# TonyLianLong/RCF-UnsupVideoSeg

Hardware: AMD Instinct MI355X
Metric: training frames/sec at 480x854 (RCF stage-1) (higher is better)
Workload: dtype f32 (3xfp16-MFMA split); 1 GPU; RCF stage-1 ResNet50+FCN train step, 8 pairs/GPU 480x854 RGB+flow, fp32, SyncBN, Adam (configs[1]); pairs_per_gpu=8, global_pairs=8, parallelism=dp1

## Files before the change

### include/rcf_hip.h

```cpp
#ifndef RCF_HIP_H
#define RCF_HIP_H
#include <stddef.h>
#include <stdint.h>

#ifdef __cplusplus
extern "C" {
#endif

#define RCF_EINVAL (-1)
#define RCF_EWORKSPACE (-2)

#define RCF_F32 0
#define RCF_BF16 1

const char *rcf_version(void);

typedef struct {
    int N, H, W, Cin;
    int Ho, Wo, Cout;
    int R, S, stride, pad, dil;
    int x_pitch, y_pitch;
    const unsigned *amax_x, *amax_w, *amax_dy;
    const void *w_pairs;
    const void *w_pairs_t;
// ... 212 lines not shown
                         const unsigned char *relu_mask, const double *sums2, const double *sums2_local, double count,
                         float *dgamma, float *dbeta, unsigned *amax_out, const unsigned *amax_x, const unsigned *amax_dy,
                         const rcf_bn_bwd_second *second, unsigned flags, void *stream);
int rcf_bn_bwd_reduce_mp(const void *dy, int ydt, int dy_pitch, const void *x, int xdt, int x_pitch, const void *y,
                         int y_pitch, long rows, int C, const float *mean, const float *invstd, int relu,
                         const unsigned char *relu_mask, const float *chan_scale, long rows_per_image, double *sums2,
                         void *workspace, size_t workspace_bytes, unsigned flags, void *stream);
int rcf_bn_bwd_apply_mp(const void *dy, int ydt, int dy_pitch, const void *x, int xdt, int x_pitch, const void *y,
                        int y_pitch, void *dx, int dx_pitch, void *dres, int dres_pitch, int res_beta, long rows, int C,
                        const float *mean, const float *invstd, const float *gamma, int relu,
                        const unsigned char *relu_mask, const float *chan_scale, long rows_per_image,
                        const double *sums2, const double *sums2_local, double count, float *dgamma, float *dbeta,
                        unsigned *amax_out, const unsigned *amax_x, const unsigned *amax_dy, unsigned flags, void *stream);
int rcf_colsum_mp(const void *x, int xdt, long rows, int C, int pitch, float *out, int beta, void *workspace,
                  size_t workspace_bytes, void *stream);

int rcf_maxpool3x3s2_fwd_f32(const float *x, float *y, uint8_t *argmax, int N, int H, int W, int C, int Ho,
                             int Wo, void *stream);
int rcf_maxpool3x3s2_bwd_f32(const float *dy, const uint8_t *argmax, float *dx, int N, int H, int W, int C,
                             int Ho, int Wo, void *stream);
int rcf_resize_bilinear_nhwc_fwd_f32(const float *x, int x_pitch, float *y, int y_pitch, int N, int Hi, int Wi,
                                     int Ho, int Wo, int C, int align_corners, void *stream);
int rcf_resize_bilinear_nhwc_bwd_f32(const float *dy, int dy_pitch, float *dx, int dx_pitch, int beta, int N,
                                     int Hi, int Wi, int Ho, int Wo, int C, int align_corners, void *stream);
int rcf_resize_bilinear_nhwc_fwd_frame_f32(const float *x, int x_pitch, float *y, int y_pitch, int N, int Hi, int Wi,
                                           int Ho, int Wo, int C, int align_corners, int frame, void *stream);
int rcf_resize_bilinear_nhwc_bwd_frame_f32(const float *dy, int dy_pitch, float *dx, int dx_pitch, int beta, int N,
                                           int Hi, int Wi, int Ho, int Wo, int C, int align_corners, int frame,
                                           void *stream);
int rcf_resize_bilinear_nchw_f32(const float *x, float *y, int planes, int Hi, int Wi, int Ho, int Wo,
// ... 184 lines not shown
```

### rcf-unsupvideoseg_amd/_lib.py

```python
import ctypes
import os
from ctypes import c_int, c_uint, c_long, c_float, c_double, c_void_p, c_size_t, c_char_p

HERE = os.path.dirname(os.path.abspath(__file__))
LIB_PATH = os.path.join(HERE, "librcf_hip.so")
LIB_PATHS = {"bf16": LIB_PATH, "f16": os.path.join(HERE, "librcf_hip_f16.so")}
ACTIVE = "bf16"


class RcfHipError(RuntimeError):
    pass


class ConvShape(ctypes.Structure):
    _fields_ = [(n, c_int) for n in ("N", "H", "W", "Cin", "Ho", "Wo", "Cout", "R", "S", "stride", "pad", "dil",
                                     "x_pitch", "y_pitch")] + \
               [(n, ctypes.c_void_p) for n in ("amax_x", "amax_w", "amax_dy", "w_pairs", "w_pairs_t", "w_pairs2",
                                                "w_pairs2_t", "amax_y")] + \
               [("flags", ctypes.c_uint), ("struct_bytes", ctypes.c_uint)]


class BnBwdIn(ctypes.Structure):
    _fields_ = [("x", ctypes.c_void_p), ("x_pitch", c_int), ("relu_mask", ctypes.c_void_p), ("mean", ctypes.c_void_p),
                ("invstd", ctypes.c_void_p)]
# ... 170 lines not shown
    "rcf_fill_f32": (c_int, [P, c_long, c_float, P]),
    "rcf_dropout2d_scale_f32": (c_int, [P, c_long, c_float, ctypes.c_ulonglong, P]),
    "rcf_bn_stats_mp": (c_int, [P, c_int, c_long, c_int, c_int, P, P, c_size_t, P]),
    "rcf_bn_apply_mp": (c_int, [P, c_int, c_int, P, c_int, P, c_int, c_int, c_long, c_int, P, P, P, P, c_int, P, c_long, P,
                                P, P, P, P, c_uint, P]),
    "rcf_bn_apply_res_mp": (c_int, [P, c_int, c_int, P, c_int, P, P, c_int, c_int, c_long, c_int, P, P, P, P, c_int, P, c_long, P,
                                    P, P, P, P, c_uint, P]),
    "rcf_bn_bwd_reduce2_mp": (c_int, [P, c_int, c_int, P, c_int, c_int, P, c_int, c_long, c_int, P, P, P, P, P, P, P, c_size_t, c_uint, P]),
    "rcf_bn_bwd_apply2_mp": (c_int, [P, c_int, c_int, P, c_int, c_int, P, c_int, c_long, c_int, P, P, P, P, P, P, c_double, P, P, P, P, P, P,
                                     c_uint, P]),
    "rcf_bn_bwd_reduce_mp": (c_int, [P, c_int, c_int, P, c_int, c_int, P, c_int, c_long, c_int, P, P, c_int, P, P, c_long,
                                     P, P, c_size_t, c_uint, P]),
    "rcf_bn_bwd_apply_mp": (c_int, [P, c_int, c_int, P, c_int, c_int, P, c_int, P, c_int, P, c_int, c_int, c_long, c_int, P,
                                    P, P, c_int, P, P, c_long, P, P, c_double, P, P, P, P, P, c_uint, P]),
    "rcf_colsum_mp": (c_int, [P, c_int, c_long, c_int, c_int, P, c_int, P, c_size_t, P]),
    "rcf_maxpool3x3s2_fwd_mp": (c_int, [P, P, c_int, P, c_int, c_int, c_int, c_int, c_int, c_int, P]),
    "rcf_maxpool3x3s2_bwd_mp": (c_int, [P, P, P, c_int, c_int, c_int, c_int, c_int, c_int, c_int, P]),
    "rcf_resize_bilinear_nhwc_fwd_mp": (c_int, [P, c_int, P, c_int, c_int, c_int, c_int, c_int, c_int, c_int, c_int, c_int,
                                                c_int, P]),
    "rcf_resize_bilinear_nhwc_bwd_mp": (c_int, [P, c_int, P, c_int, c_int, c_int, c_int, c_int, c_int, c_int, c_int, c_int,
                                                c_int, c_int, P]),
    "rcf_copy2d_batched_mp": (c_int, [P, c_long, c_long, c_long, P, c_long, c_long, c_long, c_int, c_long, c_int, c_int,
                                      c_int, c_int, P]),
    "rcf_copy2d_mp": (c_int, [P, c_int, c_long, P, c_int, c_long, c_long, c_int, c_int, P]),
    "rcf_split_rect_mp": (c_int, [P, P, P, c_int, c_int, c_int, c_int, c_int, c_int, c_int, c_int, c_int, P]),
    "rcf_conv_weight_bf16_bytes": (c_size_t, [c_int, c_int, c_int, c_int, c_int]),
    "rcf_conv_weight_bf16": (c_int, [P, c_int, c_int, c_int, c_int, c_int, P, c_uint, P]),
    "rcf_conv2d_fwd_stats_bf16_workspace_bytes": (c_size_t, [_CS]),
    "rcf_conv2d_fwd_bf16": (c_int, [P, P, P, P, c_int, _CS, _CR, c_int, c_float, c_int, P, P, c_size_t, P]),
    "rcf_conv2d_dgrad_bf16_workspace_bytes": (c_size_t, [_CS]),
# ... 63 lines not shown
```

### rcf-unsupvideoseg_amd/backbone.py

```python
import torch
import torch.nn as nn

from . import layers, ops
from .layers import (Act, BatchNorm2d, Conv2d, commuted_concat_conv, commuted_concat_conv_ok, concat_channels,
                     maxpool3x3s2)


def make_norm(norm_cfg, n):
    t = (norm_cfg or {}).get("type", "BN")
    if t not in ("BN", "SyncBN"):
        raise NotImplementedError(f"norm type {t}")
    return BatchNorm2d(n, requires_grad=bool((norm_cfg or {}).get("requires_grad", True)), sync=(t == "SyncBN"))


class Downsample(nn.Module):

    def __init__(self, conv, norm):
        super().__init__()
        self.add_module("0", conv)
        self.add_module("1", norm)

    def fwd(self, x, tape, dist, lazy=False):
        conv, norm = getattr(self, "0"), getattr(self, "1")
        if layers.fold_ok(conv, norm, x):
# ... 90 lines not shown
        if pretrained is not None:
            raise NotImplementedError("load checkpoints through load_state_dict (main.py:76-144 does)")
        for m in self.modules():
            if isinstance(m, Conv2d):
                nn.init.kaiming_normal_(m.weight, a=0, mode="fan_out", nonlinearity="relu")
            elif isinstance(m, BatchNorm2d):
                nn.init.constant_(m.weight, 1)
                nn.init.constant_(m.bias, 0)
        if self.zero_init_residual:
            for m in self.modules():
                if isinstance(m, Bottleneck):
                    nn.init.constant_(m.bn3.weight, 0)

    def fwd(self, img, tape, dist=None):
        tape.mark("stem")
        x = self.bn1.fwd(self.conv1.fwd(img, tape, stats=self.bn1.stats_request(dist)), tape, relu=True, dist=dist)
        x = maxpool3x3s2(x, tape)
        outs = []
        for i in range(self.num_stages):
            tape.mark(f"layer{i + 1}")
            nxt = getattr(getattr(self, f"layer{i + 2}"), "0").takes_planes(tape.act_dtype) if i + 1 < self.num_stages else self.heads_take_planes
            x = getattr(self, f"layer{i + 1}").fwd(x, tape, dist, next_takes_planes=nxt)
            if i in self.out_indices:
                outs.append(x)
        return outs

    def forward(self, x):
        from .layers import Tape
        img = Act(ops.nchw_to_nhwc(x.contiguous().float(), 4), needs_grad=False)
        outs = self.fwd(img, Tape(enabled=False))
        return tuple(ops.nhwc_to_nchw(o.t) for o in outs)

# ... 86 lines not shown
```

### rcf-unsupvideoseg_amd/config.py

```python
import argparse
import os

import yaml


class _UniqueKeyLoader(yaml.SafeLoader):
    def construct_mapping(self, node, deep=False):
        seen = set()
        for key_node, _ in node.value:
            key = self.construct_object(key_node, deep=deep)
            if key in seen:
                raise ValueError(f"Duplicate {key!r} key found in YAML.")
            seen.add(key)
        return super().construct_mapping(node, deep)


def _merge(base, new):
    for k, v in new.items():
        if isinstance(v, dict) and isinstance(base.get(k), dict):
            _merge(base[k], v)
        else:
            base[k] = v
    return base

# ... 122 lines not shown
        if name == "stage22_soft":
            kw["pl_mask_pos_th"] = -1
        oc = 2
    elif name == "freeze":
        kw = stage1_model_kwargs(ms, dropout=0.0, norm=norm)
        kw["freeze_backbone"] = True
    else:
        raise KeyError(name)
    kw.update(log_interval=10 ** 9, train_iter=1)
    return kw, oc


class Schedule:

    __slots__ = ("overlap_wgrad", "late_wgrad", "side_priority", "overlap_teacher", "fuse_bn_stats", "fuse_bn_finalize",
                 "fuse_bn_bwd", "relu_bitmask", "defer_residual", "lazy_downsample_norm", "merge_downsample_bwd", "fold_bn", "fold_max_k", "fold_masked_dgrad", "fp16_pairs",
                 "h2_kinds", "planes", "join_planes", "nt_stores", "bf16_stem", "autocast_fp16_as_bf16", "cache_weight_operands", "bulk_weight_prep", "grad_group",
                 "teacher_group")

    def __init__(self):
        self.overlap_wgrad = self.late_wgrad = self.overlap_teacher = True
        self.side_priority = 0
        self.fuse_bn_stats = self.fuse_bn_finalize = self.relu_bitmask = self.defer_residual = self.lazy_downsample_norm = True
        self.merge_downsample_bwd = True
        self.fuse_bn_bwd = False
        self.fold_bn, self.fold_max_k, self.fold_masked_dgrad = True, 512, True
        self.fp16_pairs, self.h2_kinds, self.planes, self.join_planes = True, "fdw", True, "stage"
        self.bf16_stem = self.cache_weight_operands = self.bulk_weight_prep = True
        self.grad_group, self.teacher_group = "auto", False
        self.nt_stores = 0
        self.autocast_fp16_as_bf16 = False

    def set(self, **kw):
        old = {k: getattr(self, k) for k in kw}
        for k, v in kw.items():
            setattr(self, k, v)
        return old

    def parse(self, items):
# ... 11 lines not shown
```

### rcf-unsupvideoseg_amd/csrc/bn.hip

```cpp
#include "rcf_common.h"

#include <type_traits>

namespace {

constexpr int RED_THREADS = 256;

struct Sweep {
    int mode, group;
    long band;
    __device__ __forceinline__ long positions(long rows) const { return mode ? 8 * band : rows; }
    __device__ __forceinline__ long row(long l) const {
        if (!mode) return l;
        const long g = l / group, w = l - g * group;
        const long b = g & 7, pos = g >> 3, per = band / group;
        return b * band + (mode == 2 ? per - 1 - pos : pos) * group + w;
    }
};
Sweep make_sweep(int mode, long rows, int group, long row_bytes, unsigned flags) {
    Sweep s{0, 1, 0};
    if ((flags & RCF_BN_SWEEP_OFF) || mode == 0 || group <= 0 || 128 % group || rows < 8 * 1024 ||
        (!(flags & RCF_BN_SWEEP_ALWAYS) && rows * row_bytes < (192L << 20)))
        return s;
    const long mtiles = (rows + 127) / 128, mtiles8 = (mtiles + 7) / 8;
// ... 182 lines not shown
template <typename XT, int V>
struct StatsOp {
    const XT *x;
    int pitch;
    __device__ void init(int) {}
    __device__ void operator()(long r, int c0, float (&o)[2][V]) const {
        const fvec<V> v = ldv<XT, V>(x + r * pitch + c0);
#pragma unroll
        for (int e = 0; e < V; ++e) {
            o[0][e] = v.q[e >> 2][e & 3];
            o[1][e] = o[0][e] * o[0][e];
        }
    }
};

template <typename XT, typename YT, int V>
struct BwdOp {
    const YT *dy;
    const XT *x;
    const YT *y;
    const float *mean, *invstd, *scale;
    int dy_pitch, x_pitch, y_pitch, relu, C;
    long rows_per_image;
    const unsigned char *mask;
    fvec<V> mu, is;
    __device__ void init(int c0) {
        mu = ldv<float, V>(mean + c0);
        is = ldv<float, V>(invstd + c0);
    }
    __device__ void operator()(long r, int c0, float (&o)[2][V]) const {
        fvec<V> g = ldv<YT, V>(dy + r * dy_pitch + c0);
        const fvec<V> xv = ldv<XT, V>(x + r * x_pitch + c0);
        if (scale) scale_by_image<V>(g, scale, r, rows_per_image, C, c0);
        if (relu) relu_bwd<YT, V>(g, mask, y, y_pitch, r, C, c0);
#pragma unroll
        for (int e = 0; e < V; ++e) {
            const int h = e >> 2, k = e & 3;
            o[0][e] = g.q[h][k];
            o[1][e] = g.q[h][k] * ((xv.q[h][k] - mu.q[h][k]) * is.q[h][k]);
        }
    }
};

template <typename XT, typename YT, int V>
struct BwdOp2 {
    const YT *dy;
    const XT *x, *x2;
// ... 242 lines not shown
            if constexpr (PL != 2) stv<YT, V>(y + r * y_pitch + c0, o);
            if constexpr (PL != 0) {
#pragma unroll
                for (int h = 0; h < V / 4; ++h) pl_store4(planes + r * (4L * C), C, c0 + 4 * h, o.q[h], pls);
            } else {
                absmax_bits<V>(mx, o);
            }
        };
        walk_rows<RowXR<V>>(sw, rows, rpb, th.ry, finish, load_x, load_res);
    }
    if constexpr (PL == 0) {
        if (amax) block_amax(mx, amax);
    }
}

template <int V>
struct BwdNorm {
    fvec<V> mu, is, ga, sg, sgx;
    __device__ __forceinline__ BwdNorm(const float *__restrict__ mean, const float *__restrict__ invstd, const float *__restrict__ gamma,
                                       const double *__restrict__ sums2, double count, int C, int c0)
        : mu(ldv<float, V>(mean + c0)), is(ldv<float, V>(invstd + c0)), ga(ldv<float, V>(gamma + c0)) {
        const float inv_count = (float)(1.0 / count);
#pragma unroll
        for (int e = 0; e < V; ++e) {
            sg.q[e >> 2][e & 3] = (float)sums2[c0 + e] * inv_count;
            sgx.q[e >> 2][e & 3] = (float)sums2[C + c0 + e] * inv_count;
        }
    }
    __device__ __forceinline__ fvec<V> dx(const fvec<V> &g, const fvec<V> &xv) const {
        fvec<V> o;
// ... 26 lines not shown
}
template <typename XT, int V, int PL>
__device__ __forceinline__ void store_dx(XT *__restrict__ dx, int dx_pitch, long r, int C, int c0, const fvec<V> &o, float pls,
                                         unsigned &mx) {
    if constexpr (PL != 0) {
#pragma unroll
        for (int h = 0; h < V / 4; ++h) pl_store4(reinterpret_cast<char *>(dx) + r * (4L * C), C, c0 + 4 * h, o.q[h], pls);
    } else {
        stv<XT, V>(dx + r * dx_pitch + c0, o);
        absmax_bits<V>(mx, o);
    }
}
template <int V> struct RowGX { fvec<V> g, x; };
template <int V> struct RowGXX { fvec<V> g, x, w; };

template <typename XT, typename YT, int V, int PL>
__global__ void __launch_bounds__(256) bn_bwd_apply_kernel(
    const YT *__restrict__ dy, int dy_pitch, const XT *__restrict__ x, int x_pitch, const YT *__restrict__ y,
    int y_pitch, XT *__restrict__ dx, int dx_pitch, YT *__restrict__ dres, int dres_pitch, int res_beta,
    long rows, int C, int cvt, int rpb, const float *__restrict__ mean, const float *__restrict__ invstd,
    const float *__restrict__ gamma, int relu, const float *__restrict__ scale, long rows_per_image,
    const double *__restrict__ sums2, const double *__restrict__ sums2_param, double count,
    float *__restrict__ dgamma, float *__restrict__ dbeta, const unsigned char *__restrict__ mask,
    unsigned *__restrict__ amax, Sweep sw, const unsigned *__restrict__ amax_x, const unsigned *__restrict__ amax_dy, long nscale) {
    float pls = 1.f;
    if constexpr (PL != 0) {
        float smax = 1.f;
        if (scale) {
            float m = 0.f;
            for (long i = threadIdx.x; i < nscale; i += 256) m = fmaxf(m, fabsf(scale[i]));
            smax = block_max_f(m);
        }
        pls = bwd_planes_scale(mean, invstd, gamma, sums2, C, count, __uint_as_float(*amax_x), __uint_as_float(*amax_dy) * smax, amax);
    }
    add_param_grads(sums2_param, C, dgamma, dbeta);
    unsigned mx = 0u;
    const EwThread th = ew_thread<V>(C, cvt, rpb);
    if (th.active) {
        const int c0 = th.c0;
        const BwdNorm<V> nm(mean, invstd, gamma, sums2, count, C, c0);
        auto load = [&](long r, RowGX<V> &in) { in = RowGX<V>{ldv<YT, V>(dy + r * dy_pitch + c0), ldv<XT, V>(x + r * x_pitch + c0)}; };
        auto finish = [&](long r, const RowGX<V> &in) {
            fvec<V> g = in.g;
            if (scale) scale_by_image<V>(g, scale, r, rows_per_image, C, c0);
            if (relu) relu_bwd<YT, V>(g, mask, y, y_pitch, r, C, c0);
            store_dx<XT, V, PL>(dx, dx_pitch, r, C, c0, nm.dx(g, in.x), pls, mx);
            if (dres) {
                YT *dr = dres + r * dres_pitch + c0;
                if (res_beta) {
                    const fvec<V> old = ldv<YT, V>(dr);
#pragma unroll
                    for (int h = 0; h < V / 4; ++h) g.q[h] += old.q[h];
                }
                stv<YT, V>(dr, g);
            }
        };
        walk_rows<RowGX<V>>(sw, rows, rpb, th.ry, finish, load);
    }
// ... 271 lines not shown
                                    const void *y, int y_pitch, long rows, int C, const float *mean,
                                    const float *invstd, int relu, const unsigned char *relu_mask,
                                    const float *chan_scale, long rows_per_image, double *sums2, void *workspace,
                                    size_t workspace_bytes, unsigned flags, void *stream) {
    if (!dy || !x || !mean || !invstd || !sums2 || rows <= 0 || C <= 0 || C % 4) return RCF_EINVAL;
    if (relu && !y && !relu_mask) return RCF_EINVAL;
    if (dy_pitch % 4 || x_pitch % 4 || (relu && !relu_mask && y_pitch % 4)) return RCF_EINVAL;
    if (!workspace || workspace_bytes < rcf_bn_stats_workspace_bytes(rows, C)) return RCF_EWORKSPACE;
    const int V = vec_width(xdt, ydt, C, dy_pitch, x_pitch, (relu && !relu_mask) ? y_pitch : 8, 8);
    const ColGeom g = col_geom(rows, C, V);
    hipStream_t st = rcf_stream(stream);
    const int rc = dispatch(xdt, ydt, V, [&](auto xt, auto yt, auto v) {
        using XT = decltype(xt);
        using YT = decltype(yt);
        constexpr int W = decltype(v)::value;
        const BwdOp<XT, YT, W> op{(const YT *)dy, (const XT *)x, (const YT *)y, mean, invstd, chan_scale, dy_pitch, x_pitch, y_pitch,
                                  relu, C, per_image(rows_per_image), relu_mask, {}, {}};
        launch_colreduce<W, 2>(op, rows, C, g, workspace, make_sweep(2, rows, g.RG, C * dt_bytes(xdt), flags), st);
    });
    if (rc) return rc;
    RCF_LAUNCH_CHECK();
    launch_partial_sum((const double *)workspace, g.chunks, 2 * C, sums2, st);
    RCF_LAUNCH_CHECK();
    return 0;
}

extern "C" int rcf_bn_bwd_reduce_f32(const float *dy, int dy_pitch, const float *x, int x_pitch, const float *y,
                                     int y_pitch, long rows, int C, const float *mean, const float *invstd, int relu,
                                     const unsigned char *relu_mask, const float *chan_scale, long rows_per_image,
                                     double *sums2, void *workspace, size_t workspace_bytes, void *stream) {
    return rcf_bn_bwd_reduce_mp(dy, RCF_F32, dy_pitch, x, RCF_F32, x_pitch, y, y_pitch, rows, C, mean, invstd, relu,
// ... 13 lines not shown
    if (relu && !y && !relu_mask) return RCF_EINVAL;
    if (dy_pitch % 4 || x_pitch % 4 || dx_pitch % 4 || (dres && dres_pitch % 4)) return RCF_EINVAL;
    const long rpi = per_image(rows_per_image);
    const bool planes = flags & RCF_BN_DX_PLANES;
    if (planes && (xdt != RCF_F32 || ydt != RCF_F32 || C % 8 || dx_pitch != C || !amax_x || !amax_dy || !amax_out ||
                   !rcf_aligned16(dx) || (relu && !relu_mask) || (chan_scale && rows % rpi)))
        return RCF_EINVAL;
    const int V = (!(relu && !relu_mask) || y_pitch % 8 == 0) ? vec_width(xdt, ydt, C, dy_pitch, x_pitch, dx_pitch, dres ? dres_pitch : 8) : 4;
    const EwGeom g = ew_geom(rows, C / V);
    const Sweep sw = make_sweep(1, rows, g.rpb, C * dt_bytes(xdt), flags);
    const int rc = dispatch(xdt, ydt, V, [&](auto xt, auto yt, auto v) {
        using XT = decltype(xt);
        using YT = decltype(yt);
        constexpr int W = decltype(v)::value;
        auto launch = [&](auto kernel) {
            launch_elementwise(kernel, g, stream, dy, dy_pitch, x, x_pitch, y, y_pitch, dx, dx_pitch, dres, dres_pitch, res_beta, rows, C,
                               g.cvt, g.rpb, mean, invstd, gamma, relu, chan_scale, rpi, sums2, sums2_local ? sums2_local : sums2, count,
                               dgamma, dbeta, relu_mask, amax_out, sw, amax_x, amax_dy, chan_scale ? (rows / rpi) * (long)C : 0L);
        };
        if constexpr (std::is_same<XT, float>::value && std::is_same<YT, float>::value) {
            if (planes) return launch(bn_bwd_apply_kernel<float, float, 4, 1>);
        }
        launch(bn_bwd_apply_kernel<XT, YT, W, 0>);
    });
    if (rc) return rc;
    RCF_LAUNCH_CHECK();
    return 0;
}

extern "C" int rcf_bn_bwd_apply_f32(const float *dy, int dy_pitch, const float *x, int x_pitch, const float *y,
                                    int y_pitch, float *dx, int dx_pitch, float *dres, int dres_pitch, int res_beta,
                                    long rows, int C, const float *mean, const float *invstd, const float *gamma,
                                    int relu, const unsigned char *relu_mask, const float *chan_scale,
                                    long rows_per_image, const double *sums2, const double *sums2_local, double count,
                                    float *dgamma, float *dbeta, unsigned *amax_out, void *stream) {
    return rcf_bn_bwd_apply_mp(dy, RCF_F32, dy_pitch, x, RCF_F32, x_pitch, y, y_pitch, dx, dx_pitch, dres, dres_pitch,
                               res_beta, rows, C, mean, invstd, gamma, relu, relu_mask, chan_scale, rows_per_image, sums2,
                               sums2_local, count, dgamma, dbeta, amax_out, nullptr, nullptr, 0u, stream);
}

extern "C" int rcf_relu_mask_copy_mp(const void *dy, int dt, int dy_pitch, const unsigned char *relu_mask, void *out, int out_pitch,
                                     long rows, int C, int beta, void *stream) {
    if (!dy || !relu_mask || !out || rows <= 0 || C <= 0 || C % 4 || dy_pitch % 4 || out_pitch % 4 || dy_pitch < C || out_pitch < C)
        return RCF_EINVAL;
    const long n = rows * (C / 4);
    const int blocks = (int)((n + 255) / 256 > 8192 ? 8192 : (n + 255) / 256);
#define RCF_CALL(T)                                                                                                  \
    hipLaunchKernelGGL((relu_mask_copy_kernel<T>), dim3(blocks), dim3(256), 0, rcf_stream(stream), (const T *)dy, dy_pitch, \
                       relu_mask, (T *)out, out_pitch, rows, C, beta)
    RCF_DISPATCH1(dt, RCF_CALL);
#undef RCF_CALL
    RCF_LAUNCH_CHECK();
    return 0;
// ... 87 lines not shown
```

### rcf-unsupvideoseg_amd/layers.py

```python
import torch
import torch.nn as nn

from . import ops




def _round_up(n, m):
    return (n + m - 1) // m * m


class Act:
    __slots__ = ("t", "grad", "needs_grad", "stats", "bn", "amax", "grad_amax", "planes", "split", "accepts_plane_grad",
                 "grad_is_planes", "stats_global", "bn_ctx", "first_reader", "grad_sums2", "pending_add", "addend_ok",
                 "relu_out", "grad_masked", "grad_colsum", "bn_in", "relu_bits", "res_norm", "res_ctx", "res_done")

    def __init__(self, t, needs_grad=True):
        self.t, self.grad, self.needs_grad = t, None, needs_grad
        self.planes, self.split, self.accepts_plane_grad, self.grad_is_planes = None, False, False, False
        self.stats_global = False
        self.stats = None
        self.bn = None
        self.amax = None
        self.grad_amax = None
        self.bn_ctx = self.first_reader = self.grad_sums2 = None
        self.pending_add, self.addend_ok = None, False
        self.relu_out, self.grad_masked, self.grad_colsum = False, False, None
        self.relu_bits = None
        self.bn_in = None
        self.res_norm = None
        self.res_ctx, self.res_done = None, False

    def range(self):
        if self.amax is None:
            self.amax = ops.absmax(self.t)
        return self.amax

    def _materialize_pending(self):
        dy, mask = self.pending_add
        self.pending_add = None
        if self.grad is None:
            self.grad = ops.relu_mask_copy(dy, mask)
        else:
            ops.relu_mask_copy(dy, mask, out=self.grad, beta=1)
        self.grad_amax = self.grad_sums2 = None

# ... 425 lines not shown
        self.num_features, self.eps, self.momentum = num_features, eps, momentum
        self.sync = sync
        self.weight = nn.Parameter(torch.ones(num_features), requires_grad=requires_grad)
        self.bias = nn.Parameter(torch.zeros(num_features), requires_grad=requires_grad)
        self.register_buffer("running_mean", torch.zeros(num_features))
        self.register_buffer("running_var", torch.ones(num_features))
        self.register_buffer("num_batches_tracked", torch.tensor(0, dtype=torch.long))

    def stats_request(self, dist=None):
        if not self.training:
            return False
        if self.sync and dist is not None and dist.on:
            return True
        return self if SCHED.fuse_bn_finalize else True

    def fwd(self, x, tape, relu, residual=None, chan_scale=None, out=None, dist=None, planes=None, lazy=False):
        xt = x.t
        lazy = lazy and SCHED.lazy_downsample_norm and not relu and residual is None and chan_scale is None and out is None and planes is None
        if not self.sync:
            dist = None
        if self.training and x.bn is not None:
            mean, invstd, count = x.bn
        elif self.training:
            local_rows = xt.shape[0] * xt.shape[1] * xt.shape[2]
            sums = x.stats if x.stats is not None else ops.bn_stats(xt)
            count = local_rows
            if dist is not None and dist.on:
                if not x.stats_global:
                    dist.allreduce_sum(sums)
                count = local_rows * dist.world
            mean, invstd = ops.bn_finalize(sums, count, self.eps, self.momentum, self.running_mean, self.running_var)
            self.num_batches_tracked += 1
        else:
            count = 0
            mean, invstd = self.running_mean, ops.bn_invstd_from_var(self.running_var, self.eps)
        rmask = None
        if relu and tape.enabled and SCHED.relu_bitmask:
            rmask = torch.empty(xt.numel() // 4, dtype=torch.uint8, device=xt.device)
        ydt = out.dtype if out is not None else (tape.act_dtype if xt.dtype == torch.float32 else xt.dtype)
        yamax = ops.new_amax(xt.device) if SCHED.fp16_pairs and ydt == torch.float32 else None
        pl = (planes if SCHED.planes and SCHED.fp16_pairs and planes in ("only", "both") and out is None and chan_scale is None and
              xt.dtype == torch.float32 and ydt == torch.float32 and x.amax is not None and xt.shape[3] % 8 == 0 and
              xt.is_contiguous() and (residual is None or residual.t.dtype == torch.float32) else None)
        if pl == "only" and (RELU_TRACE is not None or (relu and tape.enabled and rmask is None)):
            pl = "both"
        pbuf = torch.empty(tuple(xt.shape), dtype=torch.float32, device=xt.device) if pl else None
        if lazy and ydt == xt.dtype:
            y = None
            ya = Act(xt)
            ya.res_norm = (mean, invstd, self.weight.detach(), self.bias.detach())
            ya.res_ctx = (self, x, count)
            ya.amax = x.amax
        else:
            y = ops.bn_apply(xt, mean, invstd, self.weight, self.bias, relu,
                             residual=residual.t if residual is not None else None, chan_scale=chan_scale, out=out,
                             relu_mask=rmask, amax_out=yamax, out_dtype=ydt, planes=pbuf, planes_only=pl == "only",
                             amax_x=x.amax if pl else None, amax_res=residual.range() if (pl and residual is not None) else None,
                             res_norm=residual.res_norm if residual is not None else None)
            ya = Act(y if y is not None else pbuf)
            ya.amax = yamax
            ya.planes, ya.split = pbuf, pl == "only"
        if RELU_TRACE is not None and relu:
            RELU_TRACE.append(y > 0)
        if tape.enabled:
            if not self.training:
                raise RuntimeError("tape backward through eval-mode BN is not implemented")
            if not relu and residual is None and chan_scale is None and dist is not None and dist.on:
                ya.bn_in = (xt, mean, invstd)
            if relu and rmask is not None and chan_scale is None and xt.dtype == torch.float32 and ydt == torch.float32 and xt.is_contiguous():
                ya.bn_ctx = (xt, rmask, mean, invstd)

            planes_at_fwd = bool(SCHED.planes)

            def bwd():
                if ya.res_done:
                    ya.res_done = False
                    return
                relu_b, rmask_b, y_b = relu, rmask, y

                def plane_grad(xa, g):
                    return (xa.accepts_plane_grad and planes_at_fwd and xa.t.dtype == torch.float32 and xa.amax is not None
                            and g.dtype == torch.float32)
                pend = None
                if ya.res_norm is not None and ya.pending_add is not None and ya.grad is None:
                    pend = ya.take_pending()
                if pend is not None:
                    dy, rmask_b = pend
                    relu_b, y_b = True, None
                    dpl = plane_grad(x, dy)
                    ady, ya.grad_amax = ya.grad_amax, None
                    if dpl and ady is None:
# ... 53 lines not shown
                            and dy.is_contiguous()):
                        residual.pending_add = (dy, rmask)
                    else:
                        dres, rbeta = residual.grad_slot()
                        if rbeta == 0 and ady is not None and chan_scale is None:
                            residual.grad_amax = ady
                gx, _ = x.grad_slot()
                gamax = x.grad_amax = ops.new_amax(dy.device) if SCHED.fp16_pairs and xt.dtype == torch.float32 else None
                ops.bn_bwd_apply(dy, xt, y_b, mean, invstd, self.weight, relu_b, s2, count,
                                 _param_grad(self.weight) if self.weight.requires_grad else None,
                                 _param_grad(self.bias) if self.bias.requires_grad else None,
                                 dx=gx, dres=dres, res_beta=rbeta, chan_scale=chan_scale, sums2_local=s2_local,
                                 relu_mask=rmask_b, amax_out=gamax, dx_planes=dpl, amax_x=x.amax if dpl else None, amax_dy=ady)
                x.grad_is_planes = dpl
            tape.push(bwd)
        return ya


def fold_ok(conv, bn, x, residual=None):
    t = x.t
    return (SCHED.fold_bn and t.dtype in ops.H16 and conv.k == 1 and conv.stride == 1 and conv.padding == 0 and conv.bias is None
            and not conv.act and bn.training and conv.cin % 64 == 0 and conv.cin <= SCHED.fold_max_k
            and _col_tile_ok(conv.cout) and ops.relu_mask_colsum_ok(conv.cout)
            and t.is_contiguous() and bn.num_features == conv.cout
            and (residual is None or (residual.t.dtype == t.dtype and tuple(residual.t.shape[:3]) == tuple(t.shape[:3])
                                      and residual.t.shape[3] == conv.cout)))


def conv_bn_fold(conv, bn, x, tape, relu, residual=None, dist=None):
    xt, w = x.t, conv.weight
# ... 63 lines not shown
            if gx is not None:
                ops.conv2d_fwd_bf16(xt, S, negT, c0, 1, 0, 1, out=gx, beta=1)
        tape.push(bwd)
    return ya


def maxpool3x3s2(x, tape):
    y, am = ops.maxpool_fwd(x.t)
    ya = Act(y)
    ya.amax = x.amax

    def bwd():
        dy = ya.take_grad()
        if x.needs_grad:
            assert x.grad is None
            x.grad = ops.maxpool_bwd(dy, am, x.t.shape)
    tape.push(bwd)
    return ya


def resize_into(x, tape, size, align_corners, out):
    ops.resize_nhwc_fwd(x.t, size, align_corners, out=out)


def resize_act(x, tape, size, align_corners=False):
    y = Act(ops.resize_nhwc_fwd(x.t, tuple(size), align_corners))

    def bwd():
        g = y.take_grad()
        if x.needs_grad:
            gx, beta = x.grad_slot()
# ... 177 lines not shown
```

### rcf-unsupvideoseg_amd/ops.py

```python
import ctypes
import os
from ctypes import c_void_p, byref

import torch

from . import _lib
from ._lib import ConvShape, call


def _p(t):
    return None if t is None else c_void_p(t.data_ptr())


H16 = (torch.bfloat16, torch.float16)


def half():
    return torch.float16 if _lib.ACTIVE == "f16" else torch.bfloat16


class half_storage:

    def __init__(self, dtype):
        self.want = "f16" if dtype == torch.float16 else ("bf16" if dtype == torch.bfloat16 else None)
# ... 713 lines not shown
    Ho, Wo = (H - 1) // 2 + 1, (W - 1) // 2 + 1
    y = torch.empty((N, Ho, Wo, C), dtype=x.dtype, device=x.device)
    am = torch.empty((N, Ho, Wo, C), dtype=torch.uint8, device=x.device)
    call("rcf_maxpool3x3s2_fwd_mp", _p(x), _p(y), _dt(x), _p(am), N, H, W, C, Ho, Wo, _stream())
    return y, am


def maxpool_bwd(dy, am, xshape):
    N, H, W, C = xshape
    assert dy.is_contiguous()
    dx = torch.empty(tuple(xshape), dtype=dy.dtype, device=dy.device)
    call("rcf_maxpool3x3s2_bwd_mp", _p(dy), _p(am), _p(dx), _dt(dy), N, H, W, C, dy.shape[1], dy.shape[2], _stream())
    return dx


def resize_nhwc_fwd(x, size, align_corners=False, out=None, frame=0):
    N, Hi, Wi, C = x.shape
    Ho, Wo = size
    if out is None:
        out = torch.empty((N, Ho, Wo, C), dtype=x.dtype, device=x.device)
    call("rcf_resize_bilinear_nhwc_fwd_mp", _p(x), pitch_of(x), _p(out), pitch_of(out), _same_dt(x, out), N, Hi, Wi, Ho, Wo,
         C, int(align_corners), int(frame), _stream())
    return out


def resize_nhwc_bwd(dy, in_size, align_corners=False, out=None, beta=0, frame=0):
    N, Ho, Wo, C = dy.shape
    Hi, Wi = in_size
    if out is None:
        out = torch.empty((N, Hi, Wi, C), dtype=dy.dtype, device=dy.device)
# ... 253 lines not shown
```

Before: 154.9 frames/s.

## Fuse stem BN+ReLU with 3x3 maxpool in forward and backward

Adds a kernel that applies BN, ReLU and the 3x3 stride-2 maxpool in one pass, so the full-resolution post-ReLU stem activation is never written. The backward pass gathers pooled gradients through the argmax codes directly inside the BN backward reduce and apply kernels, recomputing the ReLU from x instead of materialising a full-resolution gradient. This removes several full-size stem-tensor reads and writes, at the cost of recomputing the BN affine from x and doing gather loads with code compares in backward.

```diff
diff --git a/include/rcf_hip.h b/include/rcf_hip.h
--- a/include/rcf_hip.h
+++ b/include/rcf_hip.h
@@ -250,6 +250,16 @@
                         unsigned *amax_out, const unsigned *amax_x, const unsigned *amax_dy, unsigned flags, void *stream);
 int rcf_colsum_mp(const void *x, int xdt, long rows, int C, int pitch, float *out, int beta, void *workspace,
                   size_t workspace_bytes, void *stream);
+int rcf_bn_relu_maxpool_mp(const void *x, int xdt, void *pooled, int ydt, uint8_t *argmax, int N, int H, int W, int C, int Ho,
+                           int Wo, const float *mean, const float *invstd, const float *gamma, const float *beta,
+                           unsigned *amax_out, unsigned char *relu_mask, void *stream);
+int rcf_bn_bwd_reduce_pool_mp(const void *dpool, const uint8_t *argmax, int ydt, const void *x, int xdt, int x_pitch, int N, int H,
+                              int W, int C, int Ho, int Wo, const float *mean, const float *invstd, const float *gamma,
+                              const float *beta, double *sums2, void *workspace, size_t workspace_bytes, unsigned flags, void *stream);
+int rcf_bn_bwd_apply_pool_mp(const void *dpool, const uint8_t *argmax, int ydt, const void *x, int xdt, int x_pitch, void *dx,
+                             int dx_pitch, int N, int H, int W, int C, int Ho, int Wo, const float *mean, const float *invstd,
+                             const float *gamma, const float *beta, const double *sums2, const double *sums2_local,
+                             double count, float *dgamma, float *dbeta, unsigned *amax_out, unsigned flags, void *stream);
 
 int rcf_maxpool3x3s2_fwd_f32(const float *x, float *y, uint8_t *argmax, int N, int H, int W, int C, int Ho,
                              int Wo, void *stream);
diff --git a/rcf-unsupvideoseg_amd/_lib.py b/rcf-unsupvideoseg_amd/_lib.py
--- a/rcf-unsupvideoseg_amd/_lib.py
+++ b/rcf-unsupvideoseg_amd/_lib.py
@@ -208,6 +208,10 @@
     "rcf_bn_bwd_apply_mp": (c_int, [P, c_int, c_int, P, c_int, c_int, P, c_int, P, c_int, P, c_int, c_int, c_long, c_int, P,
                                     P, P, c_int, P, P, c_long, P, P, c_double, P, P, P, P, P, c_uint, P]),
     "rcf_colsum_mp": (c_int, [P, c_int, c_long, c_int, c_int, P, c_int, P, c_size_t, P]),
+    "rcf_bn_relu_maxpool_mp": (c_int, [P, c_int, P, c_int, P] + [c_int] * 6 + [P, P, P, P, P, P, P]),
+    "rcf_bn_bwd_reduce_pool_mp": (c_int, [P, P, c_int, P, c_int, c_int] + [c_int] * 6 + [P, P, P, P, P, P, c_size_t, c_uint, P]),
+    "rcf_bn_bwd_apply_pool_mp": (c_int, [P, P, c_int, P, c_int, c_int, P, c_int] + [c_int] * 6 + [P, P, P, P, P, P, c_double, P, P, P,
+                                                                                                   c_uint, P]),
     "rcf_maxpool3x3s2_fwd_mp": (c_int, [P, P, c_int, P, c_int, c_int, c_int, c_int, c_int, c_int, P]),
     "rcf_maxpool3x3s2_bwd_mp": (c_int, [P, P, P, c_int, c_int, c_int, c_int, c_int, c_int, c_int, P]),
     "rcf_resize_bilinear_nhwc_fwd_mp": (c_int, [P, c_int, P, c_int, c_int, c_int, c_int, c_int, c_int, c_int, c_int, c_int,
diff --git a/rcf-unsupvideoseg_amd/backbone.py b/rcf-unsupvideoseg_amd/backbone.py
--- a/rcf-unsupvideoseg_amd/backbone.py
+++ b/rcf-unsupvideoseg_amd/backbone.py
@@ -2,8 +2,7 @@
 import torch.nn as nn
 
 from . import layers, ops
-from .layers import (Act, BatchNorm2d, Conv2d, commuted_concat_conv, commuted_concat_conv_ok, concat_channels,
-                     maxpool3x3s2)
+from .layers import Act, BatchNorm2d, Conv2d, commuted_concat_conv, commuted_concat_conv_ok, concat_channels
 
 
 def make_norm(norm_cfg, n):
@@ -128,8 +127,8 @@
 
     def fwd(self, img, tape, dist=None):
         tape.mark("stem")
-        x = self.bn1.fwd(self.conv1.fwd(img, tape, stats=self.bn1.stats_request(dist)), tape, relu=True, dist=dist)
-        x = maxpool3x3s2(x, tape)
+        x = self.bn1.fwd(self.conv1.fwd(img, tape, stats=self.bn1.stats_request(dist)), tape, relu=True, dist=dist,
+                         pool=True)
         outs = []
         for i in range(self.num_stages):
             tape.mark(f"layer{i + 1}")
diff --git a/rcf-unsupvideoseg_amd/config.py b/rcf-unsupvideoseg_amd/config.py
--- a/rcf-unsupvideoseg_amd/config.py
+++ b/rcf-unsupvideoseg_amd/config.py
@@ -160,7 +160,7 @@
 class Schedule:
 
     __slots__ = ("overlap_wgrad", "late_wgrad", "side_priority", "overlap_teacher", "fuse_bn_stats", "fuse_bn_finalize",
-                 "fuse_bn_bwd", "relu_bitmask", "defer_residual", "lazy_downsample_norm", "merge_downsample_bwd", "fold_bn", "fold_max_k", "fold_masked_dgrad", "fp16_pairs",
+                 "fuse_bn_bwd", "relu_bitmask", "defer_residual", "lazy_downsample_norm", "merge_downsample_bwd", "stem_pool_fwd", "stem_pool_bwd", "fold_bn", "fold_max_k", "fold_masked_dgrad", "fp16_pairs",
                  "h2_kinds", "planes", "join_planes", "nt_stores", "bf16_stem", "autocast_fp16_as_bf16", "cache_weight_operands", "bulk_weight_prep", "grad_group",
                  "teacher_group")
 
@@ -169,6 +169,7 @@
         self.side_priority = 0
         self.fuse_bn_stats = self.fuse_bn_finalize = self.relu_bitmask = self.defer_residual = self.lazy_downsample_norm = True
         self.merge_downsample_bwd = True
+        self.stem_pool_fwd = self.stem_pool_bwd = True
         self.fuse_bn_bwd = False
         self.fold_bn, self.fold_max_k, self.fold_masked_dgrad = True, 512, True
         self.fp16_pairs, self.h2_kinds, self.planes, self.join_planes = True, "fdw", True, "stage"
diff --git a/rcf-unsupvideoseg_amd/csrc/bn.hip b/rcf-unsupvideoseg_amd/csrc/bn.hip
--- a/rcf-unsupvideoseg_amd/csrc/bn.hip
+++ b/rcf-unsupvideoseg_amd/csrc/bn.hip
@@ -220,23 +220,96 @@
     }
 };
 
-template <typename XT, typename YT, int V>
+template <typename YT, int V>
+struct DenseGrad {
+    const YT *dy;
+    int pitch;
+    __device__ __forceinline__ void init(int) {}
+    __device__ __forceinline__ fvec<V> load(long r, int c0) const { return ldv<YT, V>(dy + r * pitch + c0); }
+    __device__ __forceinline__ void relu(fvec<V> &, const fvec<V> &) const {}
+};
+template <typename YT, int V>
+struct PoolGrad {
+    const YT *dpool;
+    const uint8_t *code;
+    const float *mean, *invstd, *gamma, *beta;
+    int H, W, Ho, Wo, C;
+    fvec<V> mu, is, ga, be;
+    __device__ __forceinline__ void init(int c0) {
+        mu = ldv<float, V>(mean + c0); is = ldv<float, V>(invstd + c0);
+        ga = ldv<float, V>(gamma + c0); be = ldv<float, V>(beta + c0);
+    }
+    __device__ __forceinline__ void relu(fvec<V> &g, const fvec<V> &xv) const {
+#pragma unroll
+        for (int e = 0; e < V; ++e) {
+            const int h = e >> 2, k = e & 3;
+            g.q[h][k] = (xv.q[h][k] - mu.q[h][k]) * is.q[h][k] * ga.q[h][k] + be.q[h][k] > 0.f ? g.q[h][k] : 0.f;
+        }
+    }
+    __device__ __forceinline__ fvec<V> load(long r, int c0) const {
+        const int HW = H * W;
+        const long n = r <= 0x7fffffffL ? (long)((unsigned)r / (unsigned)HW) : r / HW;
+        const int rem = (int)(r - n * HW), yi = rem / W, xi = rem - yi * W;
+        const int oy = yi & 1, ox = xi & 1;
+        const int ry[2] = {1 - oy, 2}, rx[2] = {1 - ox, 2};
+        const int wy[2] = {(yi + 1) >> 1, (yi - 1) >> 1}, wx[2] = {(xi + 1) >> 1, (xi - 1) >> 1};
+        const bool vy[2] = {wy[0] < Ho, oy != 0}, vx[2] = {wx[0] < Wo, ox != 0};
+        fvec<V> g[4];
+        uchar4 cd[4][V / 4];
+#pragma unroll
+        for (int k = 0; k < 4; ++k) {
+#pragma unroll
+            for (int h = 0; h < V / 4; ++h) {
+                g[k].q[h] = f32x4{0.f, 0.f, 0.f, 0.f};
+                cd[k][h] = make_uchar4(255, 255, 255, 255);
+            }
+            if (vy[k >> 1] && vx[k & 1]) {
+                const long o = ((n * Ho + wy[k >> 1]) * Wo + wx[k & 1]) * C + c0;
+                g[k] = ldv<YT, V>(dpool + o);
+#pragma unroll
+                for (int h = 0; h < V / 4; ++h) cd[k][h] = *reinterpret_cast<const uchar4 *>(code + o + 4 * h);
+            }
+        }
+        fvec<V> acc;
+#pragma unroll
+        for (int h = 0; h < V / 4; ++h) acc.q[h] = f32x4{0.f, 0.f, 0.f, 0.f};
+#pragma unroll
+        for (int k = 0; k < 4; ++k) {
+            const unsigned want = ry[k >> 1] * 3 + rx[k & 1];
+#pragma unroll
+            for (int h = 0; h < V / 4; ++h) {
+                const unsigned c4[4] = {cd[k][h].x, cd[k][h].y, cd[k][h].z, cd[k][h].w};
+#pragma unroll
+                for (int e = 0; e < 4; ++e) acc.q[h][e] = c4[e] == want ? acc.q[h][e] + g[k].q[h][e] : acc.q[h][e];
+            }
+        }
+        if constexpr (!std::is_same<YT, float>::value) {
+#pragma unroll
+            for (int e = 0; e < V; ++e) acc.q[e >> 2][e & 3] = (float)(YT)acc.q[e >> 2][e & 3];
+        }
+        return acc;
+    }
+};
+
+template <typename XT, typename YT, int V, class GS = DenseGrad<YT, V>>
 struct BwdOp {
-    const YT *dy;
+    GS dy;
     const XT *x;
     const YT *y;
     const float *mean, *invstd, *scale;
-    int dy_pitch, x_pitch, y_pitch, relu, C;
+    int x_pitch, y_pitch, relu, C;
     long rows_per_image;
     const unsigned char *mask;
     fvec<V> mu, is;
     __device__ void init(int c0) {
         mu = ldv<float, V>(mean + c0);
         is = ldv<float, V>(invstd + c0);
+        dy.init(c0);
     }
     __device__ void operator()(long r, int c0, float (&o)[2][V]) const {
-        fvec<V> g = ldv<YT, V>(dy + r * dy_pitch + c0);
+        fvec<V> g = dy.load(r, c0);
         const fvec<V> xv = ldv<XT, V>(x + r * x_pitch + c0);
+        dy.relu(g, xv);
         if (scale) scale_by_image<V>(g, scale, r, rows_per_image, C, c0);
         if (relu) relu_bwd<YT, V>(g, mask, y, y_pitch, r, C, c0);
 #pragma unroll
@@ -509,6 +582,67 @@
     }
 }
 
+template <typename XT, typename YT>
+__global__ void __launch_bounds__(256) bn_relu_maxpool_kernel(const XT *__restrict__ x, YT *__restrict__ pooled,
+                                                              uint8_t *__restrict__ am, int N, int H, int W, int C, int Ho, int Wo,
+                                                              const float *__restrict__ mean, const float *__restrict__ invstd,
+                                                              const float *__restrict__ gamma, const float *__restrict__ beta,
+                                                              unsigned *__restrict__ amax, unsigned char *__restrict__ mask) {
+    const int CV = C >> 2, tx = (Wo + 3) >> 2, ty = (Ho + 3) >> 2;
+    const long total = (long)N * ty * tx * 16 * CV, step = (long)gridDim.x * blockDim.x;
+    unsigned mx = 0u;
+    for (long i = (long)blockIdx.x * blockDim.x + threadIdx.x; i < total; i += step) {
+        const int cv = (int)(i % CV);
+        long t = i / CV;
+        const int in_tile = (int)(t & 15);
+        t >>= 4;
+        const int bx = (int)(t % tx);
+        t /= tx;
+        const int by = (int)(t % ty), n = (int)(t / ty);
+        const int yo = by * 4 + (in_tile >> 2), xo = bx * 4 + (in_tile & 3);
+        if (yo >= Ho || xo >= Wo) continue;
+        const int c0 = cv * 4;
+        const f32x4 mu = ld4(mean + c0), is = ld4(invstd + c0), ga = ld4(gamma + c0), be = ld4(beta + c0);
+        f32x4 best = {-INFINITY, -INFINITY, -INFINITY, -INFINITY};
+        int bi[4] = {-1, -1, -1, -1};
+        f32x4 tap[9];
+#pragma unroll
+        for (int k = 0; k < 9; ++k) {
+            const int yi = min(max(yo * 2 - 1 + k / 3, 0), H - 1), xi = min(max(xo * 2 - 1 + k % 3, 0), W - 1);
+            tap[k] = ld4(x + (((long)n * H + yi) * W + xi) * C + c0);
+        }
+#pragma unroll
+        for (int r = 0; r < 3; ++r) {
+            const int yi = yo * 2 - 1 + r;
+            if (yi < 0 || yi >= H) continue;
+#pragma unroll
+            for (int s = 0; s < 3; ++s) {
+                const int xi = xo * 2 - 1 + s;
+                if (xi < 0 || xi >= W) continue;
+                const f32x4 xv = tap[r * 3 + s];
+                unsigned sign = 0u;
+#pragma unroll
+                for (int e = 0; e < 4; ++e) {
+                    float v = (xv[e] - mu[e]) * is[e] * ga[e] + be[e];
+                    v = v > 0.f ? v : 0.f;
+                    mx = max(mx, __float_as_uint(v));
+                    sign |= (unsigned)(v > 0.f) << e;
+                    if constexpr (!std::is_same<YT, float>::value) v = (float)(YT)v;
+                    if (bi[e] < 0 || v > best[e] || v != v) {
+                        best[e] = v;
+                        bi[e] = r * 3 + s;
+                    }
+                }
+                if (mask && r >= 1 && s >= 1) mask[(((long)n * H + yi) * W + xi) * CV + cv] = (unsigned char)sign;
+            }
+        }
+        const long o = ((((long)n * Ho + yo) * Wo + xo) * CV + cv) * 4;
+        st4(pooled + o, best);
+        *reinterpret_cast<uchar4 *>(am + o) = make_uchar4((uint8_t)bi[0], (uint8_t)bi[1], (uint8_t)bi[2], (uint8_t)bi[3]);
+    }
+    if (amax) block_amax(mx, amax);
+}
+
 template <int V>
 struct BwdNorm {
     fvec<V> mu, is, ga, sg, sgx;
@@ -565,9 +699,9 @@
 template <int V> struct RowGX { fvec<V> g, x; };
 template <int V> struct RowGXX { fvec<V> g, x, w; };
 
-template <typename XT, typename YT, int V, int PL>
+template <typename XT, typename YT, int V, int PL, class GS = DenseGrad<YT, V>>
 __global__ void __launch_bounds__(256) bn_bwd_apply_kernel(
-    const YT *__restrict__ dy, int dy_pitch, const XT *__restrict__ x, int x_pitch, const YT *__restrict__ y,
+    GS dy, const XT *__restrict__ x, int x_pitch, const YT *__restrict__ y,
     int y_pitch, XT *__restrict__ dx, int dx_pitch, YT *__restrict__ dres, int dres_pitch, int res_beta,
     long rows, int C, int cvt, int rpb, const float *__restrict__ mean, const float *__restrict__ invstd,
     const float *__restrict__ gamma, int relu, const float *__restrict__ scale, long rows_per_image,
@@ -590,9 +724,11 @@
     if (th.active) {
         const int c0 = th.c0;
         const BwdNorm<V> nm(mean, invstd, gamma, sums2, count, C, c0);
-        auto load = [&](long r, RowGX<V> &in) { in = RowGX<V>{ldv<YT, V>(dy + r * dy_pitch + c0), ldv<XT, V>(x + r * x_pitch + c0)}; };
+        dy.init(c0);
+        auto load = [&](long r, RowGX<V> &in) { in = RowGX<V>{dy.load(r, c0), ldv<XT, V>(x + r * x_pitch + c0)}; };
         auto finish = [&](long r, const RowGX<V> &in) {
             fvec<V> g = in.g;
+            dy.relu(g, in.x);
             if (scale) scale_by_image<V>(g, scale, r, rows_per_image, C, c0);
             if (relu) relu_bwd<YT, V>(g, mask, y, y_pitch, r, C, c0);
             store_dx<XT, V, PL>(dx, dx_pitch, r, C, c0, nm.dx(g, in.x), pls, mx);
@@ -894,7 +1030,7 @@
         using XT = decltype(xt);
         using YT = decltype(yt);
         constexpr int W = decltype(v)::value;
-        const BwdOp<XT, YT, W> op{(const YT *)dy, (const XT *)x, (const YT *)y, mean, invstd, chan_scale, dy_pitch, x_pitch, y_pitch,
+        const BwdOp<XT, YT, W> op{{(const YT *)dy, dy_pitch}, (const XT *)x, (const YT *)y, mean, invstd, chan_scale, x_pitch, y_pitch,
                                   relu, C, per_image(rows_per_image), relu_mask, {}, {}};
         launch_colreduce<W, 2>(op, rows, C, g, workspace, make_sweep(2, rows, g.RG, C * dt_bytes(xdt), flags), st);
     });
@@ -938,7 +1074,8 @@
         using YT = decltype(yt);
         constexpr int W = decltype(v)::value;
         auto launch = [&](auto kernel) {
-            launch_elementwise(kernel, g, stream, dy, dy_pitch, x, x_pitch, y, y_pitch, dx, dx_pitch, dres, dres_pitch, res_beta, rows, C,
+            launch_elementwise(kernel, g, stream, DenseGrad<YT, W>{(const YT *)dy, dy_pitch}, x, x_pitch, y, y_pitch, dx, dx_pitch, dres,
+                               dres_pitch, res_beta, rows, C,
                                g.cvt, g.rpb, mean, invstd, gamma, relu, chan_scale, rpi, sums2, sums2_local ? sums2_local : sums2, count,
                                dgamma, dbeta, relu_mask, amax_out, sw, amax_x, amax_dy, chan_scale ? (rows / rpi) * (long)C : 0L);
         };
@@ -961,6 +1098,80 @@
     return rcf_bn_bwd_apply_mp(dy, RCF_F32, dy_pitch, x, RCF_F32, x_pitch, y, y_pitch, dx, dx_pitch, dres, dres_pitch,
                                res_beta, rows, C, mean, invstd, gamma, relu, relu_mask, chan_scale, rows_per_image, sums2,
                                sums2_local, count, dgamma, dbeta, amax_out, nullptr, nullptr, 0u, stream);
+}
+
+static bool pool_dims_ok(int N, int H, int W, int C, int Ho, int Wo) {
+    return N > 0 && H > 0 && W > 0 && C > 0 && C % 4 == 0 && Ho == (H - 1) / 2 + 1 && Wo == (W - 1) / 2 + 1 && (long)H * W <= 0x7fffffffL;
+}
+
+extern "C" int rcf_bn_relu_maxpool_mp(const void *x, int xdt, void *pooled, int ydt, uint8_t *argmax, int N, int H, int W, int C,
+                                      int Ho, int Wo, const float *mean, const float *invstd, const float *gamma, const float *beta,
+                                      unsigned *amax_out, unsigned char *relu_mask, void *stream) {
+    if (!x || !pooled || !argmax || !mean || !invstd || !gamma || !beta || !pool_dims_ok(N, H, W, C, Ho, Wo)) return RCF_EINVAL;
+    const long total = (long)N * ((Ho + 3) / 4) * ((Wo + 3) / 4) * 16 * (C / 4);
+    const long blocks = (total + 255) / 256;
+#define RCF_CALL(XT, YT)                                                                                                         \
+    hipLaunchKernelGGL((bn_relu_maxpool_kernel<XT, YT>), dim3((unsigned)(blocks > 8192 ? 8192 : blocks)), dim3(256), 0,           \
+                       rcf_stream(stream), (const XT *)x, (YT *)pooled, argmax, N, H, W, C, Ho, Wo, mean, invstd, gamma, beta,  \
+                       amax_out, relu_mask)
+    RCF_DISPATCH2(xdt, ydt, RCF_CALL);
+#undef RCF_CALL
+    RCF_LAUNCH_CHECK();
+    return 0;
+}
+
+extern "C" int rcf_bn_bwd_reduce_pool_mp(const void *dpool, const uint8_t *argmax, int ydt, const void *x, int xdt, int x_pitch, int N,
+                                         int H, int W, int C, int Ho, int Wo, const float *mean, const float *invstd,
+                                         const float *gamma, const float *beta, double *sums2, void *workspace, size_t workspace_bytes, unsigned flags,
+                                         void *stream) {
+    if (!dpool || !argmax || !x || !mean || !invstd || !gamma || !beta || !sums2 || !pool_dims_ok(N, H, W, C, Ho, Wo) || x_pitch % 4 || x_pitch < C)
+        return RCF_EINVAL;
+    const long rows = (long)N * H * W;
+    if (!workspace || workspace_bytes < rcf_bn_stats_workspace_bytes(rows, C)) return RCF_EWORKSPACE;
+    const int V = vec_width(xdt, ydt, C, C, x_pitch, 8, 8);
+    const ColGeom g = col_geom(rows, C, V);
+    hipStream_t st = rcf_stream(stream);
+    const int rc = dispatch(xdt, ydt, V, [&](auto xt, auto yt, auto v) {
+        using XT = decltype(xt);
+        using YT = decltype(yt);
+        constexpr int W_ = decltype(v)::value;
+        using GS = PoolGrad<YT, W_>;
+        const BwdOp<XT, YT, W_, GS> op{GS{(const YT *)dpool, argmax, mean, invstd, gamma, beta, H, W, Ho, Wo, C, {}, {}, {}, {}}, (const XT *)x, nullptr, mean, invstd,
+                                       nullptr, x_pitch, 0, 0, C, 1, nullptr, {}, {}};
+        launch_colreduce<W_, 2>(op, rows, C, g, workspace, make_sweep(2, rows, g.RG, C * dt_bytes(xdt), flags), st);
+    });
+    if (rc) return rc;
+    RCF_LAUNCH_CHECK();
+    launch_partial_sum((const double *)workspace, g.chunks, 2 * C, sums2, st);
+    RCF_LAUNCH_CHECK();
+    return 0;
+}
+
+extern "C" int rcf_bn_bwd_apply_pool_mp(const void *dpool, const uint8_t *argmax, int ydt, const void *x, int xdt, int x_pitch, void *dx,
+                                        int dx_pitch, int N, int H, int W, int C, int Ho, int Wo, const float *mean,
+                                        const float *invstd, const float *gamma, const float *beta, const double *sums2,
+                                        const double *sums2_local, double count, float *dgamma, float *dbeta, unsigned *amax_out,
+                                        unsigned flags, void *stream) {
+    if (!dpool || !argmax || !x || !dx || !mean || !invstd || !gamma || !beta || !sums2 || !pool_dims_ok(N, H, W, C, Ho, Wo) || count <= 0 ||
+        x_pitch % 4 || dx_pitch % 4 || x_pitch < C || dx_pitch < C || (flags & RCF_BN_DX_PLANES))
+        return RCF_EINVAL;
+    const long rows = (long)N * H * W;
+    const int V = vec_width(xdt, ydt, C, C, x_pitch, dx_pitch, 8);
+    const EwGeom g = ew_geom(rows, C / V);
+    const Sweep sw = make_sweep(1, rows, g.rpb, C * dt_bytes(xdt), flags);
+    const int rc = dispatch(xdt, ydt, V, [&](auto xt, auto yt, auto v) {
+        using XT = decltype(xt);
+        using YT = decltype(yt);
+        constexpr int W_ = decltype(v)::value;
+        using GS = PoolGrad<YT, W_>;
+        launch_elementwise(bn_bwd_apply_kernel<XT, YT, W_, 0, GS>, g, stream, GS{(const YT *)dpool, argmax, mean, invstd, gamma, beta, H, W, Ho, Wo, C, {}, {}, {}, {}},
+                           x, x_pitch, (const void *)nullptr, 0, dx, dx_pitch, (void *)nullptr, 0, 0, rows, C, g.cvt, g.rpb, mean, invstd, gamma,
+                           0, (const float *)nullptr, 1L, sums2, sums2_local ? sums2_local : sums2, count, dgamma, dbeta,
+                           (const unsigned char *)nullptr, amax_out, sw, (const unsigned *)nullptr, (const unsigned *)nullptr, 0L);
+    });
+    if (rc) return rc;
+    RCF_LAUNCH_CHECK();
+    return 0;
 }
 
 extern "C" int rcf_relu_mask_copy_mp(const void *dy, int dt, int dy_pitch, const unsigned char *relu_mask, void *out, int out_pitch,
diff --git a/rcf-unsupvideoseg_amd/layers.py b/rcf-unsupvideoseg_amd/layers.py
--- a/rcf-unsupvideoseg_amd/layers.py
+++ b/rcf-unsupvideoseg_amd/layers.py
@@ -13,7 +13,7 @@
 class Act:
     __slots__ = ("t", "grad", "needs_grad", "stats", "bn", "amax", "grad_amax", "planes", "split", "accepts_plane_grad",
                  "grad_is_planes", "stats_global", "bn_ctx", "first_reader", "grad_sums2", "pending_add", "addend_ok",
-                 "relu_out", "grad_masked", "grad_colsum", "bn_in", "relu_bits", "res_norm", "res_ctx", "res_done")
+                 "relu_out", "grad_masked", "grad_colsum", "bn_in", "relu_bits", "res_norm", "res_ctx", "res_done", "pool_ok", "pool_grad")
 
     def __init__(self, t, needs_grad=True):
         self.t, self.grad, self.needs_grad = t, None, needs_grad
@@ -30,6 +30,7 @@
         self.bn_in = None
         self.res_norm = None
         self.res_ctx, self.res_done = None, False
+        self.pool_ok, self.pool_grad = False, None
 
     def range(self):
         if self.amax is None:
@@ -485,7 +486,7 @@
             return True
         return self if SCHED.fuse_bn_finalize else True
 
-    def fwd(self, x, tape, relu, residual=None, chan_scale=None, out=None, dist=None, planes=None, lazy=False):
+    def fwd(self, x, tape, relu, residual=None, chan_scale=None, out=None, dist=None, planes=None, lazy=False, pool=False):
         xt = x.t
         lazy = lazy and SCHED.lazy_downsample_norm and not relu and residual is None and chan_scale is None and out is None and planes is None
         if not self.sync:
@@ -505,10 +506,15 @@
         else:
             count = 0
             mean, invstd = self.running_mean, ops.bn_invstd_from_var(self.running_var, self.eps)
+        ydt = out.dtype if out is not None else (tape.act_dtype if xt.dtype == torch.float32 else xt.dtype)
+        pool_through = bool(pool and relu and SCHED.stem_pool_bwd and residual is None and chan_scale is None and xt.is_contiguous()
+                            and xt.dtype == torch.float32 and ydt == torch.float32)
+        pool_fused = bool(pool and relu and SCHED.stem_pool_fwd and residual is None and chan_scale is None and out is None
+                          and planes is None and not lazy and RELU_TRACE is None and xt.is_contiguous()
+                          and (not tape.enabled or (self.training and (pool_through or SCHED.relu_bitmask))))
         rmask = None
-        if relu and tape.enabled and SCHED.relu_bitmask:
+        if relu and tape.enabled and SCHED.relu_bitmask and not (pool_fused and pool_through):
             rmask = torch.empty(xt.numel() // 4, dtype=torch.uint8, device=xt.device)
-        ydt = out.dtype if out is not None else (tape.act_dtype if xt.dtype == torch.float32 else xt.dtype)
         yamax = ops.new_amax(xt.device) if SCHED.fp16_pairs and ydt == torch.float32 else None
         pl = (planes if SCHED.planes and SCHED.fp16_pairs and planes in ("only", "both") and out is None and chan_scale is None and
               xt.dtype == torch.float32 and ydt == torch.float32 and x.amax is not None and xt.shape[3] % 8 == 0 and
@@ -516,7 +522,14 @@
         if pl == "only" and (RELU_TRACE is not None or (relu and tape.enabled and rmask is None)):
             pl = "both"
         pbuf = torch.empty(tuple(xt.shape), dtype=torch.float32, device=xt.device) if pl else None
-        if lazy and ydt == xt.dtype:
+        pool_src = None
+        if pool_fused:
+            y = None
+            pooled, codes = ops.bn_relu_maxpool(xt, mean, invstd, self.weight, self.bias, out_dtype=ydt, amax_out=yamax, relu_mask=rmask)
+            pool_src = (codes,)
+            ya = Act(pooled)
+            ya.amax = yamax
+        elif lazy and ydt == xt.dtype:
             y = None
             ya = Act(xt)
             ya.res_norm = (mean, invstd, self.weight.detach(), self.bias.detach())
@@ -540,12 +553,35 @@
                 ya.bn_in = (xt, mean, invstd)
             if relu and rmask is not None and chan_scale is None and xt.dtype == torch.float32 and ydt == torch.float32 and xt.is_contiguous():
                 ya.bn_ctx = (xt, rmask, mean, invstd)
+            ya.pool_ok = pool_through and not pool_fused
 
             planes_at_fwd = bool(SCHED.planes)
 
             def bwd():
                 if ya.res_done:
                     ya.res_done = False
+                    return
+                pg = None
+                if pool_src is not None and pool_through:
+                    pg = (ya.take_grad(),) + pool_src
+                elif pool_src is not None:
+                    ya.grad = ops.maxpool_bwd(ya.take_grad(), pool_src[0], xt.shape)
+                elif ya.pool_grad is not None:
+                    pg, ya.pool_grad = ya.pool_grad, None
+                    assert ya.grad is None and ya.pending_add is None
+                if pg is not None:
+                    s2 = ops.bn_bwd_reduce_pool(*pg, xt, mean, invstd, self.weight, self.bias)
+                    s2_local = None
+                    if dist is not None and dist.on:
+                        s2_local = s2.clone()
+                        _exchange_sums2(dist, s2, None, None)
+                    gx, _ = x.grad_slot()
+                    gamax = x.grad_amax = ops.new_amax(xt.device) if SCHED.fp16_pairs and xt.dtype == torch.float32 else None
+                    ops.bn_bwd_apply_pool(*pg, xt, mean, invstd, self.weight, self.bias, s2, count,
+                                          _param_grad(self.weight) if self.weight.requires_grad else None,
+                                          _param_grad(self.bias) if self.bias.requires_grad else None, dx=gx, sums2_local=s2_local,
+                                          amax_out=gamax)
+                    x.grad_is_planes = False
                     return
                 relu_b, rmask_b, y_b = relu, rmask, y
 
@@ -629,6 +665,8 @@
                                  relu_mask=rmask_b, amax_out=gamax, dx_planes=dpl, amax_x=x.amax if dpl else None, amax_dy=ady)
                 x.grad_is_planes = dpl
             tape.push(bwd)
+        if pool and not pool_fused:
+            return maxpool3x3s2(ya, tape)
         return ya
 
 
@@ -722,7 +760,10 @@
         dy = ya.take_grad()
         if x.needs_grad:
             assert x.grad is None
-            x.grad = ops.maxpool_bwd(dy, am, x.t.shape)
+            if x.pool_ok and SCHED.stem_pool_bwd:
+                x.pool_grad = (dy, am)
+            else:
+                x.grad = ops.maxpool_bwd(dy, am, x.t.shape)
     tape.push(bwd)
     return ya
 
diff --git a/rcf-unsupvideoseg_amd/ops.py b/rcf-unsupvideoseg_amd/ops.py
--- a/rcf-unsupvideoseg_amd/ops.py
+++ b/rcf-unsupvideoseg_amd/ops.py
@@ -751,6 +751,39 @@
     return dx
 
 
+def bn_relu_maxpool(x, mean, invstd, gamma, beta, out_dtype=None, amax_out=None, relu_mask=None):
+    _need_cuda(x)
+    N, H, W, C = x.shape
+    assert x.is_contiguous()
+    Ho, Wo = (H - 1) // 2 + 1, (W - 1) // 2 + 1
+    y = torch.empty((N, Ho, Wo, C), dtype=out_dtype or x.dtype, device=x.device)
+    am = torch.empty((N, Ho, Wo, C), dtype=torch.uint8, device=x.device)
+    call("rcf_bn_relu_maxpool_mp", _p(x), _dt(x), _p(y), _dt(y), _p(am), N, H, W, C, Ho, Wo, _p(mean), _p(invstd), _p(gamma), _p(beta),
+         _p(amax_out), _p(relu_mask), _stream())
+    return y, am
+
+
+def bn_bwd_reduce_pool(dpool, am, x, mean, invstd, gamma, beta):
+    N, H, W, C = x.shape
+    assert dpool.is_contiguous() and am.is_contiguous() and tuple(dpool.shape) == tuple(am.shape)
+    sums2 = torch.empty(2 * C, dtype=torch.float64, device=x.device)
+    need = _lib.load().rcf_bn_stats_workspace_bytes(N * H * W, C)
+    ws = workspace(need, x.device)
+    call("rcf_bn_bwd_reduce_pool_mp", _p(dpool), _p(am), _dt(dpool), _p(x), _dt(x), pitch_of(x), N, H, W, C,
+         dpool.shape[1], dpool.shape[2], _p(mean), _p(invstd), _p(gamma), _p(beta), _p(sums2), _p(ws), need, BN_FLAGS, _stream())
+    return sums2
+
+
+def bn_bwd_apply_pool(dpool, am, x, mean, invstd, gamma, beta, sums2, count, dgamma, dbeta, dx=None, sums2_local=None, amax_out=None):
+    N, H, W, C = x.shape
+    if dx is None:
+        dx = torch.empty(tuple(x.shape), dtype=x.dtype, device=x.device)
+    call("rcf_bn_bwd_apply_pool_mp", _p(dpool), _p(am), _dt(dpool), _p(x), _same_dt(x, dx), pitch_of(x), _p(dx),
+         pitch_of(dx), N, H, W, C, dpool.shape[1], dpool.shape[2], _p(mean), _p(invstd), _p(gamma), _p(beta), _p(sums2), _p(sums2_local), float(count),
+         _p(dgamma), _p(dbeta), _p(amax_out), BN_FLAGS, _stream())
+    return dx
+
+
 def resize_nhwc_fwd(x, size, align_corners=False, out=None, frame=0):
     N, Hi, Wi, C = x.shape
     Ho, Wo = size
```

New measurement: 154.7 frames/s. No clear change (-0.1%).
